# google-research/weatherbench2

Hardware: AMD Instinct MI355X
Metric: grid-point-evals/sec (721x1440x13) (higher is better)
Workload: dtype f32 (elementwise) + f64 (sums); 1 GPU; BASELINE configs[1]: 721x1440x13 f32, deterministic MSE+RMSE+MAE+Bias+ACC, 13 predefined slice regions, running init-time mean; pool_units=48, regions=13, rows_per_chunk=32, step=one wb2_det_suite_step call (K1 + K2 + time accumulate), parallelism=init-time shards x1, 1 all-reduce of [sum,count], launcher=single process

## Files before the change

include/wb2hip.h:

```cpp
#ifndef WB2HIP_H_
#define WB2HIP_H_

#include <stdint.h>

#ifdef __cplusplus
extern "C" {
#endif

#define WB2_VERSION 1

#define WB2_F32 0
#define WB2_F64 1

#define WB2_MODE_DET 0
#define WB2_MODE_DET_ACC 1
#define WB2_MODE_WIND 2

#define WB2_MODE_ENS 3

#define WB2_MODE_GAUSS 4
#define WB2_MODE_GAUSS_THR 5
#define WB2_MODE_SEEPS 7
#define WB2_MODE_ENS_THR 6

// ... 266 lines not shown
                               double* partials, int64_t arena_offset);
int wb2_program_add_gather(void* program, int32_t input, int64_t first,
                           int64_t count, int32_t source, int64_t step_bytes,
                           int32_t value_offset, const int32_t* cell,
                           const int64_t* base);
int wb2_program_add_sink(void* program, const int32_t* src,
                         const uint8_t* round32, int64_t n_out, int64_t n_time,
                         int skipna, const int32_t* sel, const int64_t* rsz8,
                         int64_t max_rows);
int wb2_program_finalize(void* program, double* arena, int32_t n_ptrs,
                         int32_t n_values);
int wb2_program_replay(void* program, const int64_t* ptrs, int32_t n_ptrs,
                       const int64_t* values, int32_t n_values,
                       const int64_t* sink_args, const int64_t* rows,
                       int32_t n_rows, void* stream);
int wb2_program_stats(void* program, double* seconds, int64_t* replays);

int wb2_energy_layout(int32_t n_member, int skipna, int has_wfield,
                      int32_t* block, int32_t* n_block, int32_t* n_slot);
int wb2_energy_score(int dtype, int skipna, const void* ens,
                     const int64_t* ens_slab, const void* truth,
                     const int64_t* truth_slab, int32_t n_member,
                     int64_t member_stride, int64_t n_outer,
                     const wb2_plan_tables* plan, double* partials,
                     double* means, double* out, void* stream);

int wb2_spatial_accumulate_addr(int dtype, int skipna, int aligned16,
                                const int64_t* f_addr, const int64_t* t_addr,
                                int64_t n_time, int64_t n_dst, int64_t n_point,
                                const int64_t* sum_addr,
// ... 262 lines not shown
```

weatherbench2_amd/_lib.py:

```python
from __future__ import annotations

import ctypes
import os

import torch

from weatherbench2_amd import build as _build

WB2_F32, WB2_F64 = 0, 1
MODE_DET, MODE_DET_ACC, MODE_WIND, MODE_ENS, MODE_GAUSS = 0, 1, 2, 3, 4
MODE_GAUSS_THR, MODE_ENS_THR, MODE_SEEPS = 5, 6, 7
GENERIC_KQ = {MODE_GAUSS: 2, MODE_GAUSS_THR: 3, MODE_ENS_THR: 4,
              MODE_SEEPS: 1}
NMETRIC = 5
NMETRIC_ENS = 8
METRIC_INDEX = {'mse': 0, 'rmse': 1, 'mae': 2, 'bias': 3, 'acc': 4}
ENS_METRIC_INDEX = {'crps': 0, 'crps_spread': 1, 'crps_skill': 2,
                    'ensemble_mean_mse': 3, 'ensemble_mean_rmse': 4,
                    'ensemble_variance': 5, 'ensemble_stddev': 6,
                    'debiased_ensemble_mean_mse': 7}

_c = ctypes
_vp, _i32, _i64, _int = _c.c_void_p, _c.c_int32, _c.c_int64, _c.c_int
_u64 = _c.c_uint64
# ... 51 lines not shown
    'wb2_program_create': (_int, [_c.POINTER(_vp)]),
    'wb2_program_destroy': (_int, [_vp]),
    'wb2_program_add_launch': (_int, [
        _vp, _c.POINTER(PlanTables), _int, _int, _int, _i32, _i64, _i64, _vp,
        _vp, _vp, _vp, _i64, _int]),
    'wb2_program_add_ens_launch': (_int, [
        _vp, _c.POINTER(PlanTables), _int, _int, _i32, _i64, _i64, _vp, _vp,
        _vp, _i64]),
    'wb2_program_add_gather': (_int, [_vp, _i32, _i64, _i64, _i32, _i64, _i32,
                                      _vp, _vp]),
    'wb2_program_add_sink': (_int, [_vp, _vp, _vp, _i64, _i64, _int, _vp, _vp,
                                    _i64]),
    'wb2_program_finalize': (_int, [_vp, _vp, _i32, _i32]),
    'wb2_program_replay': (_int, [_vp, _vp, _i32, _vp, _i32, _vp, _vp, _i32,
                                  _vp]),
    'wb2_program_stats': (_int, [_vp, _c.POINTER(_c.c_double),
                                 _c.POINTER(_i64)]),
    'wb2_energy_layout': (_int, [_i32, _int, _int, _c.POINTER(_i32),
                                 _c.POINTER(_i32), _c.POINTER(_i32)]),
    'wb2_energy_score': (_int, [
        _int, _int, _vp, _vp, _vp, _vp, _i32, _i64, _i64,
        _c.POINTER(PlanTables), _vp, _vp, _vp, _vp]),
    'wb2_time_accumulate': (_int, [_vp, _i64, _i64, _i64, _int, _vp, _vp,
                                   _vp]),
    'wb2_time_accumulate_scatter': (_int, [_int, _vp, _i64, _i64, _i64, _int,
                                           _vp, _vp, _vp, _vp]),
    'wb2_time_accumulate_runs': (_int, [_int, _vp, _i64, _i64, _i64, _int,
                                        _vp, _i64, _vp, _vp, _vp]),
    'wb2_ens_partials': (_int, [
        _int, _int, _vp, _vp, _vp, _vp, _i32, _i64, _i64, _i32, _i32, _vp, _vp,
# ... 202 lines not shown
```

weatherbench2_amd/csrc/program.cpp:

```cpp
#include "common.hpp"
#include "reduce_common.hpp"
#include "trace.hpp"
#include "wb2hip.h"

#include <chrono>
#include <cstring>
#include <memory>
#include <vector>

namespace wb2 {
namespace {

constexpr int kRing = 4;
constexpr int kSide = 2;

struct Gather {
  int input;
  long long first, count;
  int source;
  long long step_bytes;
  int value_offset;
  std::vector<int> cell;
  std::vector<long long> base;
};

struct Launch {
  wb2_plan_tables plan;
  int mode, dtype, skipna, n_in, side;
  bool ensemble = false;
  int n_member = 0;
  long long member_stride = 0;
  long long n_outer, n_pair;
  std::vector<int> slot;
  std::vector<long long> rel;
  std::vector<Gather> gathers;
  double* partials;
  double* wind_partials;
  long long arena_offset;
  long long table_offset;
};

struct Sink {
  const int32_t* src;
  const uint8_t* round32;
  long long n_out, n_time;
  int skipna;
  const int32_t* sel;
  const int64_t* rsz8;
};

struct Program {
  std::vector<Launch> launches;
  std::vector<Sink> sinks;
  double* arena = nullptr;
  long long table_len = 0;
  long long max_rows = 0;
  int n_ptrs = 0, n_values = 0;
  bool finalized = false;
  void* pinned[kRing] = {};
  void* device[kRing] = {};
  hipEvent_t copied[kRing] = {};
  hipEvent_t done[kRing] = {};
  bool busy[kRing] = {};
  int next = 0;
  hipStream_t copy_stream = nullptr;
  hipStream_t side[kSide] = {};
  hipEvent_t fork = nullptr, join[kSide] = {};
  bool any_side = false;
  double spent[5] = {};
  long long replays = 0;
};

inline double now_s() {
  return std::chrono::duration<double>(
             std::chrono::steady_clock::now().time_since_epoch())
      .count();
}

int release(Program* p) {
  for (int i = 0; i < kRing; ++i) {
    if (p->busy[i]) (void)hipEventSynchronize(p->done[i]);
    if (p->copied[i]) (void)hipEventDestroy(p->copied[i]);
    if (p->done[i]) (void)hipEventDestroy(p->done[i]);
    if (p->pinned[i]) (void)hipHostFree(p->pinned[i]);
    if (p->device[i]) (void)hipFree(p->device[i]);
  }
  for (int i = 0; i < kSide; ++i) {
    if (p->side[i]) {
      (void)hipStreamSynchronize(p->side[i]);
      (void)hipStreamDestroy(p->side[i]);
    }
    if (p->join[i]) (void)hipEventDestroy(p->join[i]);
  }
  if (p->fork) (void)hipEventDestroy(p->fork);
  if (p->copy_stream) (void)hipStreamDestroy(p->copy_stream);
  delete p;
  return 0;
}

}
}

extern "C" {

int wb2_program_create(void** program) {
  WB2_TRACE();
  using namespace wb2;
  WB2_REQUIRE(program != nullptr, "null pointer argument");
  *program = new Program();
// ... 27 lines not shown
  Launch la{};
  la.plan = *plan;
  la.mode = mode;
  la.dtype = dtype;
  la.skipna = skipna;
  la.n_in = n_in;
  la.side = side_stream != 0;
  la.n_outer = n_outer;
  la.n_pair = n_pair;
  const size_t n = (size_t)n_in * (size_t)n_outer;
  la.slot.assign(slot, slot + n);
  la.rel.assign(reinterpret_cast<const long long*>(rel),
                reinterpret_cast<const long long*>(rel) + n);
  for (size_t i = 0; i < n; ++i)
    WB2_REQUIRE(la.slot[i] >= 0, "negative pointer slot");
  la.partials = partials;
  la.wind_partials = wind_partials;
  la.arena_offset = arena_offset;
  la.table_offset = p->table_len;
  p->table_len += (long long)n;
  p->any_side = p->any_side || la.side;
  p->launches.push_back(std::move(la));
  return 0;
}

int wb2_program_add_ens_launch(void* program, const wb2_plan_tables* plan,
                               int dtype, int skipna, int32_t n_member,
                               int64_t member_stride, int64_t n_outer,
                               const int32_t* slot, const int64_t* rel,
                               double* partials, int64_t arena_offset) {
  WB2_TRACE();
  using namespace wb2;
// ... 11 lines not shown
  la.plan = *plan;
  la.mode = WB2_MODE_ENS;
  la.dtype = dtype;
  la.skipna = skipna;
  la.n_in = 2;
  la.ensemble = true;
  la.n_member = n_member;
  la.member_stride = member_stride;
  la.n_outer = n_outer;
  const size_t n = 2 * (size_t)n_outer;
  la.slot.assign(slot, slot + n);
  la.rel.assign(reinterpret_cast<const long long*>(rel),
                reinterpret_cast<const long long*>(rel) + n);
  for (size_t i = 0; i < n; ++i)
    WB2_REQUIRE(la.slot[i] >= 0, "negative pointer slot");
  la.partials = partials;
  la.arena_offset = arena_offset;
  la.table_offset = p->table_len;
  p->table_len += (long long)n;
  p->launches.push_back(std::move(la));
  return 0;
}

int wb2_program_add_gather(void* program, int32_t input, int64_t first,
                           int64_t count, int32_t source, int64_t step_bytes,
                           int32_t value_offset, const int32_t* cell,
                           const int64_t* base) {
  WB2_TRACE();
  using namespace wb2;
  WB2_REQUIRE(program && cell && base, "null pointer argument");
  auto* p = static_cast<Program*>(program);
// ... 53 lines not shown
  WB2_REQUIRE(program && arena, "null pointer argument");
  auto* p = static_cast<Program*>(program);
  WB2_REQUIRE(!p->finalized && !p->launches.empty(), "nothing to finalize");
  WB2_REQUIRE(n_ptrs > 0 && n_values >= 0, "bad sizes");
  for (const Launch& la : p->launches) {
    for (int s : la.slot)
      WB2_REQUIRE(s < n_ptrs, "pointer slot %d >= n_ptrs=%d", s, n_ptrs);
    for (const Gather& g : la.gathers) {
      WB2_REQUIRE(g.source < n_ptrs, "gather source out of range");
      for (int c : g.cell)
        WB2_REQUIRE(g.value_offset + c < n_values,
                    "gather cell %d beyond n_values=%d", g.value_offset + c,
                    n_values);
    }
  }
  p->arena = arena;
  p->n_ptrs = n_ptrs;
  p->n_values = n_values;
  const size_t bytes = (size_t)(p->table_len + p->max_rows) * sizeof(int64_t);
  for (int i = 0; i < kRing; ++i) {
    WB2_HIP_OK(hipHostMalloc(&p->pinned[i], bytes, hipHostMallocDefault));
    WB2_HIP_OK(hipMalloc(&p->device[i], bytes));
    WB2_HIP_OK(hipEventCreateWithFlags(&p->copied[i], hipEventDisableTiming));
    WB2_HIP_OK(hipEventCreateWithFlags(&p->done[i], hipEventDisableTiming));
  }
  WB2_HIP_OK(hipStreamCreateWithFlags(&p->copy_stream, hipStreamNonBlocking));
  if (p->any_side) {
    int least = 0, greatest = 0;
    WB2_HIP_OK(hipDeviceGetStreamPriorityRange(&least, &greatest));
    for (int i = 0; i < kSide; ++i) {
      WB2_HIP_OK(hipStreamCreateWithPriority(&p->side[i], hipStreamNonBlocking,
                                             greatest));
      WB2_HIP_OK(hipEventCreateWithFlags(&p->join[i], hipEventDisableTiming));
    }
    WB2_HIP_OK(hipEventCreateWithFlags(&p->fork, hipEventDisableTiming));
  }
  p->finalized = true;
  return 0;
}

int wb2_program_replay(void* program, const int64_t* ptrs, int32_t n_ptrs,
                       const int64_t* values, int32_t n_values,
                       const int64_t* sink_args, const int64_t* rows,
                       int32_t n_rows, void* stream) {
  WB2_TRACE();
  using namespace wb2;
  WB2_REQUIRE(program && ptrs && sink_args, "null pointer argument");
  auto* p = static_cast<Program*>(program);
  WB2_REQUIRE(p->finalized, "finalize the program first");
  WB2_REQUIRE(n_ptrs == p->n_ptrs && n_values == p->n_values &&
                  (n_values == 0 || values) && n_rows >= 0 &&
                  n_rows <= p->max_rows && (n_rows == 0 || rows),
// ... 25 lines not shown
    }
    for (size_t i = 0; i < n; ++i) low |= out[i];
    aligned[li] = (low & 15) == 0;
  }
  if (n_rows)
    std::memcpy(table + p->table_len, rows, (size_t)n_rows * sizeof(int64_t));
  const size_t bytes = (size_t)(p->table_len + n_rows) * sizeof(int64_t);
  t1 = now_s();
  p->spent[1] += t1 - t0;
  t0 = t1;
  WB2_HIP_OK(hipMemcpyAsync(p->device[r], table, bytes, hipMemcpyHostToDevice,
                            p->copy_stream));
  WB2_HIP_OK(hipEventRecord(p->copied[r], p->copy_stream));
  WB2_HIP_OK(hipStreamWaitEvent(s, p->copied[r], 0));
  p->busy[r] = true;
  t1 = now_s();
  p->spent[2] += t1 - t0;
  t0 = t1;
  const int64_t* dev = static_cast<const int64_t*>(p->device[r]);
  auto run = [&](const Launch& la, int aligned16, hipStream_t ls) -> int {
    const int64_t* slabs[4] = {nullptr, nullptr, nullptr, nullptr};
    for (int j = 0; j < la.n_in; ++j)
      slabs[j] = dev + la.table_offset + (long long)j * la.n_outer;
    double* metrics = p->arena + la.arena_offset;
    if (la.ensemble) {
      int rc = ens_partials_addr(la.plan, la.dtype, la.skipna, slabs[0],
                                 slabs[1], la.n_member, la.member_stride,
                                 la.n_outer, la.partials, ls);
      if (rc != 0) return rc;
      return combine_mode(la.plan, WB2_MODE_ENS, la.skipna, plan_nwf(la.plan),
                          la.partials, la.n_outer, nullptr, metrics, ls);
    }
    if (la.n_pair > 0) {
      const long long n_det =
          (long long)WB2_NMETRIC * la.plan.n_region * la.n_outer;
      return wb2_det_wind_suite_step(
          &la.plan, la.mode, la.dtype, la.skipna, nullptr, slabs, aligned16,
          la.n_outer, la.n_pair, la.partials, la.wind_partials, metrics,
          metrics + n_det, ls);
    }
    return wb2_det_suite_step(&la.plan, la.mode, la.dtype, la.skipna, nullptr,
                              slabs, aligned16, la.n_outer, la.partials,
                              metrics, 0, 0, 0, 0, nullptr, nullptr, nullptr,
                              ls);
  };
  int n_side = 0;
  if (p->any_side) {
    WB2_HIP_OK(hipEventRecord(p->fork, s));
    for (size_t li = 0; li < p->launches.size(); ++li) {
      const Launch& la = p->launches[li];
      if (!la.side) continue;
      hipStream_t ls = p->side[n_side % kSide];
      if (n_side < kSide) WB2_HIP_OK(hipStreamWaitEvent(ls, p->fork, 0));
      ++n_side;
      const int rc = run(la, aligned[li], ls);
      if (rc != 0) return rc;
    }
  }
  for (size_t li = 0; li < p->launches.size(); ++li) {
    const Launch& la = p->launches[li];
    if (la.side) continue;
    const int rc = run(la, aligned[li], s);
    if (rc != 0) return rc;
  }
  for (int i = 0; i < kSide && i < n_side; ++i) {
    WB2_HIP_OK(hipEventRecord(p->join[i], p->side[i]));
    WB2_HIP_OK(hipStreamWaitEvent(s, p->join[i], 0));
  }
  t1 = now_s();
  p->spent[3] += t1 - t0;
  t0 = t1;
  long long row0 = 0;
  for (size_t si = 0; si < p->sinks.size(); ++si) {
    const Sink& k = p->sinks[si];
    const int64_t* a = sink_args + 3 * si;
    const int64_t* sum_addr = reinterpret_cast<const int64_t*>(a[0]);
    const int64_t* count_addr = reinterpret_cast<const int64_t*>(a[1]);
    int rc;
    if (k.sel) {
      const long long mine = a[2];
      WB2_REQUIRE(mine >= 0 && row0 + mine <= n_rows,
                  "sink %zu: rows out of range", si);
      rc = wb2_gather_accumulate_rows(p->arena, k.src, k.round32, k.n_out,
                                      k.n_time, k.skipna, sum_addr, count_addr,
                                      dev + p->table_len + row0, k.sel, k.rsz8,
                                      s);
      row0 += mine;
    } else {
      rc = wb2_gather_accumulate(p->arena, k.src, k.round32, k.n_out, k.n_time,
                                 k.skipna, sum_addr, count_addr, s);
    }
    if (rc != 0) return rc;
  }
  WB2_HIP_OK(hipEventRecord(p->done[r], s));
  p->spent[4] += now_s() - t0;
  ++p->replays;
  return 0;
}

int wb2_program_stats(void* program, double* seconds, int64_t* replays) {
  using namespace wb2;
  WB2_REQUIRE(program && seconds && replays, "null pointer argument");
  auto* p = static_cast<Program*>(program);
  for (int i = 0; i < 5; ++i) seconds[i] = p->spent[i];
  *replays = p->replays;
  return 0;
}

}
// ... 1 lines not shown
```

weatherbench2_amd/csrc/reduce_common.hpp:

```cpp
#pragma once

#include "common.hpp"
#include "wb2hip.h"

#include <cstdint>

#ifndef WB2_ROTATE_CHUNKS
#define WB2_ROTATE_CHUNKS 1
#endif

namespace wb2 {


#define WB2_PLAN_OF_ARGS(t, field_dtype) \
  wb2_plan_tables t{};                   \
  t.n_row = n_row;                       \
  t.n_col = n_col;                       \
  t.n_chunk = n_chunk;                   \
  t.n_ctile = n_ctile;                   \
  t.n_seg = n_seg;                       \
  t.n_ts = n_ts;                         \
  t.w_row = w_row;                       \
  t.w_col = w_col;                       \
  t.wfield = wfield;                     \
// ... 51 lines not shown
  p.n_row = t.n_row;
  p.n_col = t.n_col;
  p.n_chunk = t.n_chunk;
  p.n_ctile = t.n_ctile;
  p.n_seg = t.n_seg;
  p.n_ts = t.n_ts;
}

int combine_slots(const wb2_plan_tables& t, int mode, int skipna, int k_slots,
                  int nwf, const double* partials, int64_t n_outer,
                  double* sums, double* metrics, void* stream);
int combine_mode(const wb2_plan_tables& t, int mode, int skipna, int nwf,
                 const double* partials, int64_t n_outer, double* sums,
                 double* metrics, void* stream);

int ens_partials_addr(const wb2_plan_tables& t, int dtype, int skipna,
                      const int64_t* ens_addr, const int64_t* truth_addr,
                      int32_t n_member, int64_t member_stride, int64_t n_outer,
                      double* partials, void* stream);

__device__ __forceinline__ void swap_halves32(double& a, double& b) {
  const unsigned long long ua = __builtin_bit_cast(unsigned long long, a);
  const unsigned long long ub = __builtin_bit_cast(unsigned long long, b);
  const auto lo = __builtin_amdgcn_permlane32_swap(
      (unsigned)ua, (unsigned)ub, false, false);
  const auto hi = __builtin_amdgcn_permlane32_swap(
      (unsigned)(ua >> 32), (unsigned)(ub >> 32), false, false);
  a = __builtin_bit_cast(double, ((unsigned long long)hi[0] << 32) | lo[0]);
  b = __builtin_bit_cast(double, ((unsigned long long)hi[1] << 32) | lo[1]);
}
// ... 124 lines not shown
```

weatherbench2_amd/csrc/stream_reduce.hip:

```cpp

#include "common.hpp"
#include "trace.hpp"
#include "reduce_common.hpp"
#include "gauss_math.hpp"
#include "wb2hip.h"

#include <atomic>
#include <type_traits>

namespace wb2 {
namespace {

constexpr int kMaxIn = 4;

struct StreamParams {
  const void* in[kMaxIn];
  const long long* slab[kMaxIn];
  const double* w_row;
  const double* w_col;
  const void* wfield;
  const double* aux;
  double scalar;
  const int* chunk_row0;
  const int* chunk_nrow;
// ... 1753 lines not shown
  p.K = k_slots;
  p.mode = mode;
  p.skipna = skipna != 0;
  p.group = 1;
  while (p.group < kWave &&
         (long long)t.n_band * nwf * t.n_seg * 8 * (2 * p.group) <= 1024)
    p.group *= 2;
  *lds = ((size_t)t.n_band * nwf * t.n_seg * p.K +
          (size_t)t.n_region * p.K * (1 + (size_t)t.n_band) +
          (size_t)t.n_region * ((size_t)t.n_seg + t.n_band)) *
         sizeof(double);
  return p;
}
}

int combine_det_and_wind(const wb2_plan_tables& t, int mode, int skipna,
                         const double* partials, int64_t n_outer,
                         const double* wind_partials, int64_t n_pair,
                         double* metrics, double* wind_metrics, void* stream) {
  const int nwf = plan_nwf(t);
  size_t lds_a = 0, lds_b = 0;
  const CombineParams a =
      combine_params(t, mode, skipna, wb2_num_slots(mode, skipna), nwf,
                     partials, n_outer, nullptr, metrics, &lds_a);
  const CombineParams b = combine_params(
      t, WB2_MODE_WIND, skipna, wb2_num_slots(WB2_MODE_WIND, skipna), nwf,
      wind_partials, n_pair, nullptr, wind_metrics, &lds_b);
  const size_t lds = lds_a > lds_b ? lds_a : lds_b;
  if (lds > 64 * 1024 || n_outer <= 0 || n_pair <= 0 ||
      n_outer + n_pair >= (1ll << 31) || !partials || !wind_partials ||
// ... 306 lines not shown
```

weatherbench2_amd/evaluation.py:

```python
from __future__ import annotations

import contextlib
import logging
import os
import typing as t

import numpy as np

from weatherbench2_amd import config
from weatherbench2_amd import indexing
from weatherbench2_amd import metrics as metrics_lib
from weatherbench2_amd import xarray_lite as xl


def _metric_and_region_loop(
    forecast,
    truth,
    eval_config: config.Eval,
    skipna: bool,
    compute_chunk: bool = False,
) -> xl.Dataset:
  given_forecast, given_truth = forecast, truth
  for name, dv in eval_config.derived_variables.items():
    forecast[name] = dv.compute(forecast)
# ... 128 lines not shown
      else:
        idx = torch.as_tensor(index, device=da.data.device)
        data = torch.index_select(da.data, ax, idx).reshape(shape)
    else:
      data = np.take(np.asarray(da.data), index, axis=ax).reshape(shape)
    dims = da.dims[:ax] + (init_dim, lead_dim) + da.dims[ax + 1:]
    out.data_vars[name] = xl.DataArray(data, dims, coords, name)
  return xl.like_input(out, *given)


_RUN_MIN = 256
_FIRST_ROWS_BYTES = 256 << 20
_LAZY_COUNT_MIN = 1 << 20


class _Accumulator:

  def __init__(self, dims, shape, split, device, lazy_count: bool = False):
    import torch
    self.dims, self.shape, self.split = dims, shape, split
    self.labels: list = []
    self.row_of: dict = {}
    self.dst: dict = {}
    self.pending: dict = {}
    if split is None:
      self.rest_shape = shape
      alloc = shape
    else:
      self.pos = dims.index(split)
      self.rest_shape = shape[:self.pos] + shape[self.pos + 1:]
# ... 85 lines not shown
    self.split_order = split_order
    self.comm = comm
    self._acc: dict = {}
    self._coords: dict = {}

  def _on_gpu(self) -> bool:
    import torch
    return self.device is not None and torch.device(self.device).type == 'cuda'

  def _on_gpu_or_unset(self) -> bool:
    return self.device is None or self._on_gpu()

  def add(self, chunk: xl.Dataset):
    import torch
    from weatherbench2_amd import engine
    for k, c in chunk.coords.items():
      if k != self.dim and k != self.split_dim and not (
          isinstance(c, xl.DataArray) and self.dim in c.dims):
        self._coords.setdefault(k, c)
    for name, da in chunk.data_vars.items():
      if self.dim not in da.dims:
        raise ValueError(f'{name} has no {self.dim!r} dim: {da.dims}')
      axis = da.dims.index(self.dim)
      dims = tuple(d for d in da.dims if d != self.dim)
      shape = tuple(n for d, n in zip(da.dims, da.shape) if d != self.dim)
      labels = chunk.coords.get(self.split_dim) if self.split_dim else None
      split = self.split_dim if (
          labels is not None and not isinstance(labels, xl.DataArray)
          and self.split_dim in dims) else None
      raw = da.data
# ... 90 lines not shown
        dist.get_world_size() > 1):
      everyone: list = [None] * dist.get_world_size()
      dist.all_gather_object(everyone, mine)
      for n in mine:
        out[n] = first_seen([e[n] for e in everyone if n in e])
    else:
      out = {n: first_seen([v]) for n, v in mine.items()}
    return out

  def result(self) -> xl.Dataset:
    import torch
    import torch.distributed as dist
    in_torch_group = (dist.is_available() and dist.is_initialized()
                      and dist.get_world_size() > 1)
    in_group = self.comm is not None or in_torch_group
    if in_group and not self._acc:
      raise ValueError('RunningMean.result() on a rank that accumulated '
                       'nothing: give every rank at least one chunk '
                       '(evaluate_chunks checks this up front)')
    names = sorted(self._acc)
    for n in names:
      self._acc[n].settle()
    labels = self._split_labels(names)
    def laid_out(n):
      acc = self._acc[n]
      lazy = acc._count is None and not in_group
      if acc.split is None:
        if lazy:
          return acc.total, torch.as_tensor(acc.steps([None])[0],
                                            dtype=torch.float64,
# ... 134 lines not shown
      flat[i] = row
    return out

  def storage(self, name, dims, shape, dtype) -> _KeptRows:
    acc = self._acc.get(name)
    if acc is None:
      acc = self._acc[name] = _KeptRows(dims, shape, self.key_dims(dims),
                                        self.device)
      self._dtypes[name] = dtype
    if acc.dims != tuple(dims) or acc.rest_shape != tuple(
        n for d, n in zip(dims, shape) if d not in acc.key_dims):
      raise ValueError(f'{name}: chunk layout changed {acc.dims} -> {dims}')
    return acc

  def snapshot(self):
    return ({n: (a.total.clone(), a.count.clone(), set(a.filled))
             for n, a in self._acc.items()},
            {k: dict(v) for k, v in self._rows.items()},
            {k: dict(v) for k, v in self._seen.items()})

  def restore(self, state):
    accs, rows, seen = state
    for n, (total, count, filled) in accs.items():
      a = self._acc[n]
      a.total, a.count, a.filled = total.clone(), count.clone(), set(filled)
    self._rows = {k: dict(v) for k, v in rows.items()}
    self._seen = {k: dict(v) for k, v in seen.items()}

  def add(self, chunk: xl.Dataset):
    import torch
    from weatherbench2_amd import engine
    for k, c in chunk.coords.items():
      if k not in (self.dim, self.split_dim) and not (
          isinstance(c, xl.DataArray) and any(
              d in (self.dim, self.split_dim) for d in c.dims)):
        self._coords.setdefault(k, c)
    rows_of_group: dict = {}
    for name, da in chunk.data_vars.items():
      if self.dim not in da.dims:
        raise ValueError(f'{name} has no {self.dim!r} dim: {da.dims}')
      raw = da.data
      if isinstance(raw, torch.Tensor):
        if self.device is None and raw.is_cuda:
          self.device = raw.device
        engine.order_read(raw)
        values = raw
# ... 7 lines not shown
        rows = rows_of_group[acc.key_dims] = self.rows(
            chunk, acc.key_dims).ravel()
      acc.claim(rows.tolist(), len(self._rows[acc.key_dims]), name)
      moved = values.to(acc.total.device, torch.float64).movedim(
          acc.key_pos, list(range(len(acc.key_pos))))
      moved = moved.reshape((rows.size,) + acc.rest_shape)
      index = torch.as_tensor(rows, device=acc.total.device)
      acc.total.index_copy_(0, index, moved)
      acc.count.index_fill_(0, index, 1.0)

  def result(self) -> xl.Dataset:
    import torch
    import torch.distributed as dist
    several = dist.is_available() and dist.is_initialized() and (
        dist.get_world_size() > 1)

    def final_dtype(name):
      try:
        final = torch.from_numpy(
            np.empty(0, dtype=np.dtype(self._dtypes[name]))).dtype
        return final if final.is_floating_point else None
      except TypeError:
        return None
    pieces = {}
    for name, acc in self._acc.items():
      keys = list(self._rows[acc.key_dims])
      rows = sorted(acc.filled)
      if rows:
        values = (acc.total[:len(rows)] if rows[-1] == len(rows) - 1
                  else acc.total[rows])
# ... 537 lines not shown
    labels = forecast.coords.get(lead_dim) if lead_dim else None
    if isinstance(labels, xl.DataArray):
      labels = labels.values
    key = (sig, None if labels is None else
           (np.asarray(labels).dtype.str, np.asarray(labels).tobytes()))
    pending.setdefault(key, [prog, []])[1].append((forecast, truth_chunk))
  drain()


def _verify_program(prog, forecast, truth_chunk, configs, skipna, sinks):
  import torch

  def snapshot(mean):
    if getattr(mean, 'keeps_time', False):
      return mean.snapshot()
    for acc in mean._acc.values():
      acc.settle()
    return {n: (acc.total.clone(), acc.count.clone(), list(acc.labels),
                dict(acc.row_of)) for n, acc in mean._acc.items()}

  def restore(mean, state):
    if getattr(mean, 'keeps_time', False):
      return mean.restore(state)
    for n, (total, count, labels, row_of) in state.items():
      acc = mean._acc[n]
      acc.total, acc.count = total.clone(), count.clone()
      acc.labels, acc.row_of, acc.dst = list(labels), dict(row_of), {}
  before = [snapshot(m) for m in sinks]
  prog.run(forecast, truth_chunk, configs, skipna, sinks)
  replayed = [snapshot(m) for m in sinks]
# ... 428 lines not shown
```

weatherbench2_amd/program.py:

```python
from __future__ import annotations

import os
import threading
import typing as t
import weakref

import numpy as np
import torch

from weatherbench2_amd import _lib, engine
from weatherbench2_amd import xarray_lite as xl

_THIRD = 1.0 / 3.0
_MAX_ELEMENTS = 1 << 21


class _Active(threading.local):

  def __init__(self):
    self.recorder = None


_ACTIVE = _Active()


def recorder():
  return _ACTIVE.recorder


def mode() -> str:
  return os.environ.get('WB2HIP_CHUNK_PROGRAM', '1')


class Recorder:

  def __init__(self, probe: bool = False):
    self.probe = probe
    self.launches: list = []
    self.tables: dict = {}
    self.offset = 0

  def __enter__(self):
    self._old = _ACTIVE.recorder
    _ACTIVE.recorder = self
    return self

# ... 381 lines not shown
        at += n
      out.append(fused)
      new_off += fused.n_values
    else:
      perm[old_off[i]:old_off[i] + la.n_values] = new_off + np.arange(
          la.n_values, dtype=np.int64)
      out.append(la)
      new_off += la.n_values
  return out, perm


class _NotReplayable(Exception):
  pass


REASONS: list = []
REPLAY_STATS: list = []


def _no(reason: str):
  REASONS.append(reason)
  del REASONS[:-16]
  return None


def _nan_equal(a: torch.Tensor, b: torch.Tensor) -> bool:
  if a.shape != b.shape or a.dtype != b.dtype:
    return False
  return bool(((a == b) | (torch.isnan(a) & torch.isnan(b))).all().item())

# ... 46 lines not shown
      each = np.concatenate([np.repeat(v[5], self.n_time)
                             for v in self.variables]).astype(np.uint8)
      self._kept = {'sel': dev(sel), 'rsz8': dev(rsz8), 'rest8': dev(rest8),
                    'vid': dev(vid), 'groups': groups, 'stamp': None,
                    'round': torch.as_tensor(each).to(self.device),
                    'max_rows': sum(g[1] for g in groups.values())}
      self._kept['sel32'] = self._kept['sel'].to(torch.int32)
    return self._kept

  def kept_rows(self, sink, forecast):
    k = self.kept_structure(sink)
    rows = {g: sink.rows(forecast, g).ravel() for g in k['groups']}
    accs = []
    for name, dims, shape, axis, src, _ in self.variables:
      acc = sink.storage(name, dims, shape, None)
      acc.claim(rows[acc.key_dims].tolist(), len(sink._rows[acc.key_dims]),
                name)
      accs.append(acc)
    stamp = tuple(a.total.data_ptr() for a in accs)
    if stamp != k['stamp']:
      sums = engine.upload_table(np.array(stamp, dtype=np.int64), self.device,
                                 cache=False)
      counts = engine.upload_table(
          np.array([a.count.data_ptr() for a in accs], dtype=np.int64),
          self.device, cache=False)
      k['sum0'] = sums[k['vid']] + k['rest8']
      k['count0'] = counts[k['vid']] + k['rest8']
      k['stamp'] = stamp
    mine = (next(iter(rows.values())) if len(rows) == 1
            else np.concatenate(list(rows.values())))
# ... 5 lines not shown
    chunk_rows = engine.upload_table(rows, self.device, cache=False)
    offset = chunk_rows[k['sel']] * k['rsz8']
    return sum0 + offset, count0 + offset, k['round']

  def reset(self):
    self._targets.clear()
    if self._kept is not None:
      self._kept['stamp'] = None

  def _accumulator_tables(self, mean, labels):
    key = None if labels is None else (labels.dtype.str, labels.tobytes())
    accs = [mean._acc[v[0]] for v in self.variables]
    hit = self._targets.get(key)
    if hit is not None and hit[0] == tuple(a.total.data_ptr() for a in accs):
      return hit[1], hit[2]
    sums, counts = [], []
    for (name, dims, shape, axis, src, _), acc in zip(self.variables, accs):
      if acc.split is not None:
        rows = acc.rows(labels)
        acc.shape = tuple(n for d, n in zip(dims, shape) if d != self.time_dim)
        dst = acc.destinations(rows)
      else:
        dst = np.arange(src.shape[0], dtype=np.int64)
      if dst.size != src.shape[0]:
        raise ValueError(f'{name}: accumulator layout changed')
      sums.append(acc.total.data_ptr() + 8 * dst)
      counts.append(acc.count.data_ptr() + 8 * dst)
    stamp = tuple(a.total.data_ptr() for a in accs)
    d_sum = engine.upload_table(np.concatenate(sums), self.device, cache=False)
    d_cnt = engine.upload_table(np.concatenate(counts), self.device,
# ... 120 lines not shown
            g.n_out * g.n_time, 1, 0, kept['sel32'].data_ptr(),
            kept['rsz8'].data_ptr(), kept['max_rows']),
                   'wb2_program_add_sink')
    self.n_ptrs = len(index_of)
    _lib.check(lib.wb2_program_finalize(handle, arena.data_ptr(), self.n_ptrs,
                                        n_values), 'wb2_program_finalize')
    self.ptrs = np.zeros(max(self.n_ptrs, 1), dtype=np.int64)
    for i, p in fixed.items():
      self.ptrs[i] = p
    self._ptrs_at = self.ptrs.ctypes.data
    self.sink_args = np.zeros((max(len(groups), 1), 3), dtype=np.int64)
    self._sink_at = self.sink_args.ctypes.data
    self._replay = lib.wb2_program_replay
    self._no_values = np.zeros(1, dtype=np.int64)
    self._values_of: dict = {}

  @staticmethod
  def _stats(lib, handle) -> dict:
    import ctypes
    sec = (ctypes.c_double * 5)()
    n = ctypes.c_int64()
    _lib.check(lib.wb2_program_stats(handle, sec, ctypes.byref(n)),
               'wb2_program_stats')
    per = max(n.value, 1)
    names = ('wait_for_slot', 'fill_table', 'copy', 'launches', 'sinks')
    out = {k: 1e3 * v / per for k, v in zip(names, sec)}
    out['replays'] = n.value
    return out

  def stats(self) -> dict:
    return self._stats(self._lib, self._handle)

  @staticmethod
  def _close(lib, handle):
    try:
      REPLAY_STATS.append(_Native._stats(lib, handle))
      del REPLAY_STATS[:-16]
    except Exception:
      pass
    lib.wb2_program_destroy(handle)

  def run(self, forecast, truth, means, stream) -> None:
    ptrs = self.ptrs
    for i, g in self.getters:
      ptrs[i] = g(forecast, truth).data_ptr()
    if self.values:
      from weatherbench2_amd import metrics as gm
      vt, dims = gm._valid_times(forecast)
      key = vt.tobytes()
      values = self._values_of.get(key)
      if values is None:
        memo: dict = {'valid_times': (forecast, vt, dims)}
        values = (self.values[0](forecast, memo) if len(self.values) == 1
                  else np.concatenate([v(forecast, memo)
                                       for v in self.values]))
        if len(self._values_of) >= 4096:
          self._values_of.clear()
# ... 6 lines not shown
        d_sum, d_cnt, mine = group.kept_rows(mean, forecast)
        rows = mine if rows is None else np.concatenate([rows, mine])
        args[k, 2] = mine.size
      else:
        labels = None
        if group.split_dim is not None:
          labels = np.asarray(forecast.coords[group.split_dim])
        d_sum, d_cnt = group._accumulator_tables(mean, labels)
      args[k, 0], args[k, 1] = d_sum.data_ptr(), d_cnt.data_ptr()
    engine.hooked_call(
        'stream_partials', self._replay, 'wb2_program_replay',
        self._handle, self._ptrs_at, self.n_ptrs, values.ctypes.data,
        self.n_values, self._sink_at,
        None if rows is None else rows.ctypes.data,
        0 if rows is None else rows.size, stream)


class ChunkProgram:

  def __init__(self, launches, groups, arena, device, time_dim, split_dim,
               means=None):
    self.launches = launches
    self.groups = groups
    self.arena = arena
    self.device = device
    self.time_dim, self.split_dim = time_dim, split_dim
    off = 0
    self.slices = []
    for la in launches:
      self.slices.append(arena[off:off + la.n_values])
# ... 85 lines not shown
    for la in launches:
      if isinstance(la, _EnsFused):
        mine[off:off + la.n_values] = True
      off += la.n_values
    pick = mine[fused_at]
    if not _nan_equal(trial[fused_at][pick], flat_real[pick]):
      _no('fused ensemble launch differs in bits: separate passes kept')
      launches, perm = singles, None
  if perm is not None:
    per_sink = [[(name, dims, shape, axis,
                  np.where(src >= 0, perm[np.maximum(src, 0)], -1), r32)
                 for name, dims, shape, axis, src, r32 in variables]
                for variables in per_sink]
  groups = [_SinkGroup(variables, device, time_dim, split_dim)
            for variables in per_sink]
  arena = torch.empty((total,), dtype=torch.float64, device=device)
  return ChunkProgram(launches, groups, arena, device, time_dim, split_dim,
                      means)


def _group_variables(shown, result, mean, forecast, flat_real, total, time_dim):
  variables = []
  for name, da in shown.data_vars.items():
    real = result.data_vars.get(name)
    if real is None or not isinstance(da.data, torch.Tensor) or not isinstance(
        real.data, torch.Tensor) or tuple(real.dims) != tuple(da.dims):
      return _no('result variable missing / not a device tensor / other dims')
    if time_dim not in da.dims:
      return _no('no time dim in a result variable')
    axis = da.dims.index(time_dim)
    v = da.data.to(torch.float64)
# ... 45 lines not shown
```

Measured before the change: 540.5 billion grid-point-evals/s.

## Run the fold and time-accumulate tail on a side lane with double-buffered arenas

Splits each replayed launch into the streaming partials pass and the fold/combine pass. When the fold groups are small, the fold and the sink accumulation go onto a high-priority side stream, with a second arena and a second set of partials alternating by replay parity. The main stream can then start the next chunk's streaming reduction while the previous tail finishes. Consumers (accumulator add, result, snapshot) now call a settle/flush that makes the current stream wait on the last tail. This adds memory, cross-stream event waits, and a risk of missing synchronisation.

```diff
diff --git a/include/wb2hip.h b/include/wb2hip.h
--- a/include/wb2hip.h
+++ b/include/wb2hip.h
@@ -304,6 +304,9 @@
                        const int64_t* values, int32_t n_values,
                        const int64_t* sink_args, const int64_t* rows,
                        int32_t n_rows, void* stream);
+int wb2_program_tail_lane(void* program, double* arena_odd,
+                          const int64_t* partials_odd, int32_t n_launches);
+int wb2_program_flush(void* program, void* stream);
 int wb2_program_stats(void* program, double* seconds, int64_t* replays);
 
 int wb2_energy_layout(int32_t n_member, int skipna, int has_wfield,
diff --git a/weatherbench2_amd/_lib.py b/weatherbench2_amd/_lib.py
--- a/weatherbench2_amd/_lib.py
+++ b/weatherbench2_amd/_lib.py
@@ -89,6 +89,8 @@
     'wb2_program_finalize': (_int, [_vp, _vp, _i32, _i32]),
     'wb2_program_replay': (_int, [_vp, _vp, _i32, _vp, _i32, _vp, _vp, _i32,
                                   _vp]),
+    'wb2_program_tail_lane': (_int, [_vp, _vp, _vp, _i32]),
+    'wb2_program_flush': (_int, [_vp, _vp]),
     'wb2_program_stats': (_int, [_vp, _c.POINTER(_c.c_double),
                                  _c.POINTER(_i64)]),
     'wb2_energy_layout': (_int, [_i32, _int, _int, _c.POINTER(_i32),
diff --git a/weatherbench2_amd/csrc/program.cpp b/weatherbench2_amd/csrc/program.cpp
--- a/weatherbench2_amd/csrc/program.cpp
+++ b/weatherbench2_amd/csrc/program.cpp
@@ -34,8 +34,8 @@
   std::vector<int> slot;
   std::vector<long long> rel;
   std::vector<Gather> gathers;
-  double* partials;
-  double* wind_partials;
+  double* partials[2];
+  double* wind_partials[2];
   long long arena_offset;
   long long table_offset;
 };
@@ -52,7 +52,9 @@
 struct Program {
   std::vector<Launch> launches;
   std::vector<Sink> sinks;
-  double* arena = nullptr;
+  double* arena[2] = {};
+  bool tail_lane = false;
+  int last = -1;
   long long table_len = 0;
   long long max_rows = 0;
   int n_ptrs = 0, n_values = 0;
@@ -66,6 +68,7 @@
   hipStream_t copy_stream = nullptr;
   hipStream_t side[kSide] = {};
   hipEvent_t fork = nullptr, join[kSide] = {};
+  hipEvent_t streamed = nullptr;
   bool any_side = false;
   double spent[5] = {};
   long long replays = 0;
@@ -75,6 +78,15 @@
   return std::chrono::duration<double>(
              std::chrono::steady_clock::now().time_since_epoch())
       .count();
+}
+
+int side_stream(Program* p, int i) {
+  if (p->side[i]) return 0;
+  int least = 0, greatest = 0;
+  WB2_HIP_OK(hipDeviceGetStreamPriorityRange(&least, &greatest));
+  WB2_HIP_OK(hipStreamCreateWithPriority(&p->side[i], hipStreamNonBlocking,
+                                         greatest));
+  return 0;
 }
 
 int release(Program* p) {
@@ -93,6 +105,7 @@
     if (p->join[i]) (void)hipEventDestroy(p->join[i]);
   }
   if (p->fork) (void)hipEventDestroy(p->fork);
+  if (p->streamed) (void)hipEventDestroy(p->streamed);
   if (p->copy_stream) (void)hipStreamDestroy(p->copy_stream);
   delete p;
   return 0;
@@ -150,8 +163,8 @@
                 reinterpret_cast<const long long*>(rel) + n);
   for (size_t i = 0; i < n; ++i)
     WB2_REQUIRE(la.slot[i] >= 0, "negative pointer slot");
-  la.partials = partials;
-  la.wind_partials = wind_partials;
+  la.partials[0] = partials;
+  la.wind_partials[0] = wind_partials;
   la.arena_offset = arena_offset;
   la.table_offset = p->table_len;
   p->table_len += (long long)n;
@@ -193,7 +206,7 @@
                 reinterpret_cast<const long long*>(rel) + n);
   for (size_t i = 0; i < n; ++i)
     WB2_REQUIRE(la.slot[i] >= 0, "negative pointer slot");
-  la.partials = partials;
+  la.partials[0] = partials;
   la.arena_offset = arena_offset;
   la.table_offset = p->table_len;
   p->table_len += (long long)n;
@@ -277,7 +290,7 @@
                     n_values);
     }
   }
-  p->arena = arena;
+  p->arena[0] = arena;
   p->n_ptrs = n_ptrs;
   p->n_values = n_values;
   const size_t bytes = (size_t)(p->table_len + p->max_rows) * sizeof(int64_t);
@@ -289,16 +302,56 @@
   }
   WB2_HIP_OK(hipStreamCreateWithFlags(&p->copy_stream, hipStreamNonBlocking));
   if (p->any_side) {
-    int least = 0, greatest = 0;
-    WB2_HIP_OK(hipDeviceGetStreamPriorityRange(&least, &greatest));
     for (int i = 0; i < kSide; ++i) {
-      WB2_HIP_OK(hipStreamCreateWithPriority(&p->side[i], hipStreamNonBlocking,
-                                             greatest));
+      if (int rc = side_stream(p, i)) return rc;
       WB2_HIP_OK(hipEventCreateWithFlags(&p->join[i], hipEventDisableTiming));
     }
     WB2_HIP_OK(hipEventCreateWithFlags(&p->fork, hipEventDisableTiming));
   }
   p->finalized = true;
+  return 0;
+}
+
+int wb2_program_tail_lane(void* program, double* arena_odd,
+                          const int64_t* partials_odd, int32_t n_launches) {
+  WB2_TRACE();
+  using namespace wb2;
+  WB2_REQUIRE(program && arena_odd && partials_odd, "null pointer argument");
+  auto* p = static_cast<Program*>(program);
+  WB2_REQUIRE(p->finalized && !p->tail_lane && p->last < 0,
+              "the tail lane is set once, after finalize and before a replay");
+  WB2_REQUIRE(arena_odd != p->arena[0], "the second arena is the first");
+  WB2_REQUIRE(n_launches == (int32_t)p->launches.size(),
+              "partials for %d launches, the program has %zu", n_launches,
+              p->launches.size());
+  for (size_t li = 0; li < p->launches.size(); ++li) {
+    const Launch& la = p->launches[li];
+    auto* part = reinterpret_cast<double*>(partials_odd[2 * li]);
+    auto* wind = reinterpret_cast<double*>(partials_odd[2 * li + 1]);
+    WB2_REQUIRE(part && part != la.partials[0] &&
+                    (la.n_pair == 0 || (wind && wind != la.wind_partials[0])),
+                "launch %zu: the second partials are missing or the first", li);
+  }
+  if (int rc = side_stream(p, 0)) return rc;
+  WB2_HIP_OK(hipEventCreateWithFlags(&p->streamed, hipEventDisableTiming));
+  for (size_t li = 0; li < p->launches.size(); ++li) {
+    Launch& la = p->launches[li];
+    la.partials[1] = reinterpret_cast<double*>(partials_odd[2 * li]);
+    la.wind_partials[1] = reinterpret_cast<double*>(partials_odd[2 * li + 1]);
+  }
+  p->arena[1] = arena_odd;
+  p->tail_lane = true;
+  return 0;
+}
+
+int wb2_program_flush(void* program, void* stream) {
+  WB2_TRACE();
+  using namespace wb2;
+  WB2_REQUIRE(program != nullptr, "null pointer argument");
+  auto* p = static_cast<Program*>(program);
+  if (p->last >= 0 && p->busy[p->last])
+    WB2_HIP_OK(hipStreamWaitEvent(static_cast<hipStream_t>(stream),
+                                  p->done[p->last], 0));
   return 0;
 }
 
@@ -354,35 +407,45 @@
   WB2_HIP_OK(hipEventRecord(p->copied[r], p->copy_stream));
   WB2_HIP_OK(hipStreamWaitEvent(s, p->copied[r], 0));
   p->busy[r] = true;
+  const int par = p->tail_lane ? (int)(p->replays & 1) : 0;
+  hipStream_t lane = p->tail_lane ? p->side[0] : s;
+  if (p->tail_lane) {
+    const int r2 = (r + kRing - 2) % kRing;
+    if (p->busy[r2]) WB2_HIP_OK(hipStreamWaitEvent(s, p->done[r2], 0));
+  }
+  double* arena = p->arena[par];
   t1 = now_s();
   p->spent[2] += t1 - t0;
   t0 = t1;
   const int64_t* dev = static_cast<const int64_t*>(p->device[r]);
-  auto run = [&](const Launch& la, int aligned16, hipStream_t ls) -> int {
+  auto stream_part = [&](const Launch& la, int aligned16,
+                         hipStream_t ls) -> int {
     const int64_t* slabs[4] = {nullptr, nullptr, nullptr, nullptr};
     for (int j = 0; j < la.n_in; ++j)
       slabs[j] = dev + la.table_offset + (long long)j * la.n_outer;
-    double* metrics = p->arena + la.arena_offset;
-    if (la.ensemble) {
-      int rc = ens_partials_addr(la.plan, la.dtype, la.skipna, slabs[0],
-                                 slabs[1], la.n_member, la.member_stride,
-                                 la.n_outer, la.partials, ls);
-      if (rc != 0) return rc;
+    if (la.ensemble)
+      return ens_partials_addr(la.plan, la.dtype, la.skipna, slabs[0], slabs[1],
+                               la.n_member, la.member_stride, la.n_outer,
+                               la.partials[par], ls);
+    return stream_step_partials(la.plan, la.mode, la.dtype, la.skipna, slabs,
+                                aligned16, la.n_outer, la.n_pair,
+                                la.partials[par], la.wind_partials[par], ls);
+  };
+  auto fold_part = [&](const Launch& la, hipStream_t ls) -> int {
+    double* metrics = arena + la.arena_offset;
+    if (la.ensemble)
       return combine_mode(la.plan, WB2_MODE_ENS, la.skipna, plan_nwf(la.plan),
-                          la.partials, la.n_outer, nullptr, metrics, ls);
-    }
+                          la.partials[par], la.n_outer, nullptr, metrics, ls);
     if (la.n_pair > 0) {
       const long long n_det =
           (long long)WB2_NMETRIC * la.plan.n_region * la.n_outer;
-      return wb2_det_wind_suite_step(
-          &la.plan, la.mode, la.dtype, la.skipna, nullptr, slabs, aligned16,
-          la.n_outer, la.n_pair, la.partials, la.wind_partials, metrics,
-          metrics + n_det, ls);
-    }
-    return wb2_det_suite_step(&la.plan, la.mode, la.dtype, la.skipna, nullptr,
-                              slabs, aligned16, la.n_outer, la.partials,
-                              metrics, 0, 0, 0, 0, nullptr, nullptr, nullptr,
-                              ls);
+      return combine_det_and_wind(la.plan, la.mode, la.skipna,
+                                  la.partials[par], la.n_outer,
+                                  la.wind_partials[par], la.n_pair, metrics,
+                                  metrics + n_det, ls);
+    }
+    return combine_mode(la.plan, la.mode, la.skipna, plan_nwf(la.plan),
+                        la.partials[par], la.n_outer, nullptr, metrics, ls);
   };
   int n_side = 0;
   if (p->any_side) {
@@ -393,19 +456,29 @@
       hipStream_t ls = p->side[n_side % kSide];
       if (n_side < kSide) WB2_HIP_OK(hipStreamWaitEvent(ls, p->fork, 0));
       ++n_side;
-      const int rc = run(la, aligned[li], ls);
+      int rc = stream_part(la, aligned[li], ls);
+      if (rc == 0 && !p->tail_lane) rc = fold_part(la, ls);
       if (rc != 0) return rc;
     }
   }
   for (size_t li = 0; li < p->launches.size(); ++li) {
     const Launch& la = p->launches[li];
     if (la.side) continue;
-    const int rc = run(la, aligned[li], s);
+    const int rc = stream_part(la, aligned[li], s);
     if (rc != 0) return rc;
   }
   for (int i = 0; i < kSide && i < n_side; ++i) {
     WB2_HIP_OK(hipEventRecord(p->join[i], p->side[i]));
     WB2_HIP_OK(hipStreamWaitEvent(s, p->join[i], 0));
+  }
+  if (p->tail_lane) {
+    WB2_HIP_OK(hipEventRecord(p->streamed, s));
+    WB2_HIP_OK(hipStreamWaitEvent(lane, p->streamed, 0));
+  }
+  for (const Launch& la : p->launches) {
+    if (la.side && !p->tail_lane) continue;
+    const int rc = fold_part(la, lane);
+    if (rc != 0) return rc;
   }
   t1 = now_s();
   p->spent[3] += t1 - t0;
@@ -421,18 +494,19 @@
       const long long mine = a[2];
       WB2_REQUIRE(mine >= 0 && row0 + mine <= n_rows,
                   "sink %zu: rows out of range", si);
-      rc = wb2_gather_accumulate_rows(p->arena, k.src, k.round32, k.n_out,
+      rc = wb2_gather_accumulate_rows(arena, k.src, k.round32, k.n_out,
                                       k.n_time, k.skipna, sum_addr, count_addr,
                                       dev + p->table_len + row0, k.sel, k.rsz8,
-                                      s);
+                                      lane);
       row0 += mine;
     } else {
-      rc = wb2_gather_accumulate(p->arena, k.src, k.round32, k.n_out, k.n_time,
-                                 k.skipna, sum_addr, count_addr, s);
+      rc = wb2_gather_accumulate(arena, k.src, k.round32, k.n_out, k.n_time,
+                                 k.skipna, sum_addr, count_addr, lane);
     }
     if (rc != 0) return rc;
   }
-  WB2_HIP_OK(hipEventRecord(p->done[r], s));
+  WB2_HIP_OK(hipEventRecord(p->done[r], lane));
+  p->last = r;
   p->spent[4] += now_s() - t0;
   ++p->replays;
   return 0;
diff --git a/weatherbench2_amd/csrc/reduce_common.hpp b/weatherbench2_amd/csrc/reduce_common.hpp
--- a/weatherbench2_amd/csrc/reduce_common.hpp
+++ b/weatherbench2_amd/csrc/reduce_common.hpp
@@ -89,6 +89,15 @@
                  const double* partials, int64_t n_outer, double* sums,
                  double* metrics, void* stream);
 
+int stream_step_partials(const wb2_plan_tables& t, int mode, int dtype,
+                         int skipna, const int64_t* const* slab,
+                         int aligned16, int64_t n_outer, int64_t n_pair,
+                         double* partials, double* wind_partials, void* stream);
+int combine_det_and_wind(const wb2_plan_tables& t, int mode, int skipna,
+                         const double* partials, int64_t n_outer,
+                         const double* wind_partials, int64_t n_pair,
+                         double* metrics, double* wind_metrics, void* stream);
+
 int ens_partials_addr(const wb2_plan_tables& t, int dtype, int skipna,
                       const int64_t* ens_addr, const int64_t* truth_addr,
                       int32_t n_member, int64_t member_stride, int64_t n_outer,
diff --git a/weatherbench2_amd/csrc/stream_reduce.hip b/weatherbench2_amd/csrc/stream_reduce.hip
--- a/weatherbench2_amd/csrc/stream_reduce.hip
+++ b/weatherbench2_amd/csrc/stream_reduce.hip
@@ -1791,6 +1791,19 @@
 }
 }
 
+int stream_step_partials(const wb2_plan_tables& t, int mode, int dtype,
+                         int skipna, const int64_t* const* slab,
+                         int aligned16, int64_t n_outer, int64_t n_pair,
+                         double* partials, double* wind_partials,
+                         void* stream) {
+  WB2_REQUIRE(slab != nullptr, "null pointer argument");
+  if (n_pair > 0)
+    return stream_pairs_impl(t, mode, dtype, skipna, nullptr, slab, aligned16,
+                             n_outer, n_pair, partials, wind_partials, stream);
+  return stream_partials_impl(t, mode, dtype, skipna, nullptr, slab, aligned16,
+                              n_outer, partials, stream);
+}
+
 int combine_det_and_wind(const wb2_plan_tables& t, int mode, int skipna,
                          const double* partials, int64_t n_outer,
                          const double* wind_partials, int64_t n_pair,
diff --git a/weatherbench2_amd/evaluation.py b/weatherbench2_amd/evaluation.py
--- a/weatherbench2_amd/evaluation.py
+++ b/weatherbench2_amd/evaluation.py
@@ -166,6 +166,11 @@
 _LAZY_COUNT_MIN = 1 << 20
 
 
+def _settle_replays() -> None:
+  from weatherbench2_amd import program
+  program.settle()
+
+
 class _Accumulator:
 
   def __init__(self, dims, shape, split, device, lazy_count: bool = False):
@@ -281,6 +286,7 @@
   def add(self, chunk: xl.Dataset):
     import torch
     from weatherbench2_amd import engine
+    _settle_replays()
     for k, c in chunk.coords.items():
       if k != self.dim and k != self.split_dim and not (
           isinstance(c, xl.DataArray) and self.dim in c.dims):
@@ -401,6 +407,7 @@
     in_torch_group = (dist.is_available() and dist.is_initialized()
                       and dist.get_world_size() > 1)
     in_group = self.comm is not None or in_torch_group
+    _settle_replays()
     if in_group and not self._acc:
       raise ValueError('RunningMean.result() on a rank that accumulated '
                        'nothing: give every rank at least one chunk '
@@ -565,6 +572,7 @@
     return acc
 
   def snapshot(self):
+    _settle_replays()
     return ({n: (a.total.clone(), a.count.clone(), set(a.filled))
              for n, a in self._acc.items()},
             {k: dict(v) for k, v in self._rows.items()},
@@ -581,6 +589,7 @@
   def add(self, chunk: xl.Dataset):
     import torch
     from weatherbench2_amd import engine
+    _settle_replays()
     for k, c in chunk.coords.items():
       if k not in (self.dim, self.split_dim) and not (
           isinstance(c, xl.DataArray) and any(
@@ -618,6 +627,7 @@
     import torch.distributed as dist
     several = dist.is_available() and dist.is_initialized() and (
         dist.get_world_size() > 1)
+    _settle_replays()
 
     def final_dtype(name):
       try:
@@ -1185,6 +1195,7 @@
   def snapshot(mean):
     if getattr(mean, 'keeps_time', False):
       return mean.snapshot()
+    _settle_replays()
     for acc in mean._acc.values():
       acc.settle()
     return {n: (acc.total.clone(), acc.count.clone(), list(acc.labels),
diff --git a/weatherbench2_amd/program.py b/weatherbench2_amd/program.py
--- a/weatherbench2_amd/program.py
+++ b/weatherbench2_amd/program.py
@@ -19,6 +19,7 @@
 
   def __init__(self):
     self.recorder = None
+    self.pending = None
 
 
 _ACTIVE = _Active()
@@ -30,6 +31,13 @@
 
 def mode() -> str:
   return os.environ.get('WB2HIP_CHUNK_PROGRAM', '1')
+
+
+def settle() -> None:
+  native = _ACTIVE.pending
+  if native is not None:
+    _ACTIVE.pending = None
+    native.flush()
 
 
 class Recorder:
@@ -441,6 +449,9 @@
   pass
 
 
+LANE_MAX_FOLD_GROUPS = 256
+
+
 REASONS: list = []
 REPLAY_STATS: list = []
 
@@ -517,6 +528,8 @@
     accs = []
     for name, dims, shape, axis, src, _ in self.variables:
       acc = sink.storage(name, dims, shape, None)
+      if len(sink._rows[acc.key_dims]) > acc.total.shape[0]:
+        settle()
       acc.claim(rows[acc.key_dims].tolist(), len(sink._rows[acc.key_dims]),
                 name)
       accs.append(acc)
@@ -552,6 +565,7 @@
     hit = self._targets.get(key)
     if hit is not None and hit[0] == tuple(a.total.data_ptr() for a in accs):
       return hit[1], hit[2]
+    settle()
     sums, counts = [], []
     for (name, dims, shape, axis, src, _), acc in zip(self.variables, accs):
       if acc.split is not None:
@@ -702,6 +716,25 @@
     self._replay = lib.wb2_program_replay
     self._no_values = np.zeros(1, dtype=np.int64)
     self._values_of: dict = {}
+    self.lane = max(la.n_total + int(getattr(la, 'n_pair', 0) or 0)
+                    for la in launches) <= LANE_MAX_FOLD_GROUPS
+    if not self.lane:
+      return
+    if arena.numel() < 2 * off:
+      raise ValueError('the arena of a native program holds the launches\' '
+                       'outputs twice')
+    odd = np.zeros((len(launches), 2), dtype=np.int64)
+    for i, la in enumerate(launches):
+      first = la if isinstance(la, _EnsPass) else la.step
+      for j, x in enumerate((first.partials,
+                             getattr(first, 'wind_partials', None))):
+        if x is not None:
+          keep.append(torch.empty_like(x))
+          odd[i, j] = keep[-1].data_ptr()
+    _lib.check(lib.wb2_program_tail_lane(
+        handle, arena.data_ptr() + 8 * off, odd.ctypes.data, len(launches)),
+               'wb2_program_tail_lane')
+    keep.append(arena)
 
   @staticmethod
   def _stats(lib, handle) -> dict:
@@ -728,7 +761,14 @@
       pass
     lib.wb2_program_destroy(handle)
 
+  def flush(self) -> None:
+    _lib.check(self._lib.wb2_program_flush(
+        self._handle, engine.current_stream_ptr(self.device)),
+               'wb2_program_flush')
+
   def run(self, forecast, truth, means, stream) -> None:
+    if _ACTIVE.pending is not self:
+      settle()
     ptrs = self.ptrs
     for i, g in self.getters:
       ptrs[i] = g(forecast, truth).data_ptr()
@@ -765,6 +805,8 @@
         self.n_values, self._sink_at,
         None if rows is None else rows.ctypes.data,
         0 if rows is None else rows.size, stream)
+    if self.lane:
+      _ACTIVE.pending = self
 
 
 class ChunkProgram:
@@ -880,7 +922,7 @@
                 for variables in per_sink]
   groups = [_SinkGroup(variables, device, time_dim, split_dim)
             for variables in per_sink]
-  arena = torch.empty((total,), dtype=torch.float64, device=device)
+  arena = torch.empty((2 * total,), dtype=torch.float64, device=device)
   return ChunkProgram(launches, groups, arena, device, time_dim, split_dim,
                       means)
 
```

Measured after the change: 540.4 billion grid-point-evals/s (median of 2 runs). About the same (-0.0%).
